# borgor/ripcurrents

Measured on AMD Instinct MI355X. Metric: frames/sec dense Farneback flow @1080p, higher is better.
Workload: dtype f32

## Files before the change

ripcurrents_amd/csrc/flow_iter_kernels.hip:

```cpp

#include <cstdlib>

#include "rc_device.h"

#define RC_ITER_BATCH 3
#define RC_RR_D 3

#ifdef RC_EXACT_BUILD
#define RC_FLOW_NS rc_flow_exact
#else
#define RC_FLOW_NS rc_flow_fast
#endif
namespace RC_FLOW_NS {

__device__ __forceinline__ float2 rc_flow_in(const RcIterArgs& a, const float2* fin, int gx, int gy) {
    if (a.in_mode == 0) return make_float2(0.f, 0.f);
    if (a.in_mode == 1) return fin[(size_t)gy * a.w + gx];
    float ax, ay;
    int sx = rc_src_x(gx, a.up_scale_x, a.fin_w, ax);
    int sx1 = min(sx + 1, a.fin_w - 1);
    int sy = rc_src_y(gy, a.up_scale_y, ay);
    int sy0 = rc_clampi(sy, 0, a.fin_h - 1), sy1 = rc_clampi(sy + 1, 0, a.fin_h - 1);
    const float2* S0 = fin + (size_t)sy0 * a.fin_w;
    const float2* S1 = fin + (size_t)sy1 * a.fin_w;
// ... 10 lines not shown
struct RcM5 { float m0, m1, m2, m3, m4; };

struct RcGather {
    float4 q00, q01, q10, q11;
    float e00, e01, e10, e11;
    float fx, fy;
    bool inside;
};

__device__ __forceinline__ void rc_gather_issue(RcGather& g, const float4* __restrict__ RA1,
                                                const float* __restrict__ RB1, int gx, int gy, float dx,
                                                float dy, int w, int h) {
    float fx = gx + dx, fy = gy + dy;
    int x1 = (int)floorf(fx), y1 = (int)floorf(fy);
    g.fx = fx - x1;
    g.fy = fy - y1;
    g.inside = (unsigned)x1 < (unsigned)(w - 1) && (unsigned)y1 < (unsigned)(h - 1);
    const size_t p = g.inside ? (size_t)y1 * w + x1 : (size_t)gy * w + gx;
    const size_t pw = g.inside ? (size_t)w : 0, p1 = g.inside ? 1 : 0;
    g.q00 = RA1[p]; g.q01 = RA1[p + p1]; g.q10 = RA1[p + pw]; g.q11 = RA1[p + pw + p1];
    g.e00 = RB1[p]; g.e01 = RB1[p + p1]; g.e10 = RB1[p + pw]; g.e11 = RB1[p + pw + p1];
}

__device__ __forceinline__ void rc_r0_prep(float4& A0, float& B0) {
#ifndef RC_EXACT_BUILD
    A0.x *= 0.5f; A0.y *= 0.5f; A0.z *= 0.5f; A0.w *= 0.5f; B0 *= 0.5f;
#endif
}

__device__ __forceinline__ RcM5 rc_matrices_reg(const float4 A0, const float B0, const RcGather& g, float dx,
                                                float dy, int X, int Y, int w, int h, bool BORDER = true) {
    float fx = g.fx, fy = g.fy;
#ifdef RC_EXACT_BUILD
    float a00 = (1.f - fx) * (1.f - fy), a01 = fx * (1.f - fy);
    float a10 = (1.f - fx) * fy, a11 = fx * fy;
#define RC_BILIN(c, e) (a00 * e##00 c + a01 * e##01 c + a10 * e##10 c + a11 * e##11 c)
    float r2 = RC_BILIN(.x, g.q), r3 = RC_BILIN(.y, g.q), r4 = RC_BILIN(.z, g.q), r5 = RC_BILIN(.w, g.q);
    float r6 = RC_BILIN(, g.e);
#undef RC_BILIN
    r4 = (A0.z + r4) * 0.5f;
    r5 = (A0.w + r5) * 0.5f;
    r6 = (B0 + r6) * 0.25f;
    if (!g.inside) {
        r2 = r3 = 0.f;
        r4 = A0.z;
        r5 = A0.w;
        r6 = B0 * 0.5f;
    }
    r2 = (A0.x - r2) * 0.5f;
    r3 = (A0.y - r3) * 0.5f;
#else
    const float hx1 = 0.5f * fx, hx0 = RC_FMA(fx, -0.5f, 0.5f), fy0 = 1.f - fy;
    const float h00 = hx0 * fy0, h01 = hx1 * fy0, h10 = hx0 * fy, h11 = hx1 * fy;
#define RC_BILIN_FROM(s0, sg, c, e) RC_FMA(sg h11, e##11 c, RC_FMA(sg h10, e##10 c, RC_FMA(sg h01, e##01 c, RC_FMA(sg h00, e##00 c, s0))))
    float r2 = RC_BILIN_FROM(A0.x, -, .x, g.q), r3 = RC_BILIN_FROM(A0.y, -, .y, g.q);
    float r4 = RC_BILIN_FROM(A0.z, +, .z, g.q), r5 = RC_BILIN_FROM(A0.w, +, .w, g.q);
    float r6 = 0.5f * RC_BILIN_FROM(B0, +, , g.e);
#undef RC_BILIN_FROM
    if (!g.inside) {
        r2 = A0.x;
        r3 = A0.y;
        r4 = 2.f * A0.z;
        r5 = 2.f * A0.w;
        r6 = B0;
    }
#endif
#ifdef RC_EXACT_BUILD
    r2 += r4 * dy + r6 * dx;
    r3 += r6 * dy + r5 * dx;
#else
    r2 = RC_FMA(r6, dx, RC_FMA(r4, dy, r2));
    r3 = RC_FMA(r5, dx, RC_FMA(r6, dy, r3));
#endif
    if (BORDER && ((unsigned)(X - 5) >= (unsigned)(w - 10) || (unsigned)(Y - 5) >= (unsigned)(h - 10))) {
        float bl = X < 5 ? (X < 2 ? 0.14f : 0.4472f) : 1.f;
        int rx = w - X - 1;
        float br = X >= w - 5 ? (rx < 2 ? 0.14f : 0.4472f) : 1.f;
        float bt = Y < 5 ? (Y < 2 ? 0.14f : 0.4472f) : 1.f;
        int ry = h - Y - 1;
        float bb = Y >= h - 5 ? (ry < 2 ? 0.14f : 0.4472f) : 1.f;
        float scale = bl * br * bt * bb;
        r2 *= scale; r3 *= scale; r4 *= scale; r5 *= scale; r6 *= scale;
    }
    RcM5 o;
#ifdef RC_EXACT_BUILD
    o.m0 = r4 * r4 + r6 * r6;
    o.m1 = (r4 + r5) * r6;
    o.m2 = r5 * r5 + r6 * r6;
    o.m3 = r4 * r2 + r6 * r3;
    o.m4 = r6 * r2 + r5 * r3;
#else
    o.m0 = RC_FMA(r4, r4, r6 * r6);
    o.m1 = (r4 + r5) * r6;
    o.m2 = RC_FMA(r5, r5, r6 * r6);
    o.m3 = RC_FMA(r4, r2, r6 * r3);
    o.m4 = RC_FMA(r6, r2, r5 * r3);
#endif
    return o;
}

__device__ __forceinline__ RcM5 rc_matrices(const float4* __restrict__ RA0, const float* __restrict__ RB0,
                                            const float4* __restrict__ RA1, const float* __restrict__ RB1,
                                            int gx, int gy, int w, int h, float dx, float dy) {
    size_t p0 = (size_t)gy * w + gx;
    float4 A0 = RA0[p0];
    float B0 = RB0[p0];
    RcGather g;
    rc_gather_issue(g, RA1, RB1, gx, gy, dx, dy, w, h);
    rc_r0_prep(A0, B0);
    return rc_matrices_reg(A0, B0, g, dx, dy, gx, gy, w, h);
}

__device__ __forceinline__ float2 rc_solve(const double* g) {
    double idet = 1. / (g[0] * g[2] - g[1] * g[1] + 1e-3);
    float2 f;
    f.x = (float)((g[0] * g[4] - g[1] * g[3]) * idet);
    f.y = (float)((g[2] * g[3] - g[1] * g[4]) * idet);
    return f;
}

__device__ __forceinline__ float rc_diff_of_products(float a, float b, float c, float d) {
    float w = c * d;
    float e = RC_FMA(-c, d, w);
    float f = RC_FMA(a, b, -w);
    return f + e;
}
__device__ __forceinline__ float2 rc_solve3(const float* g, float eps) {
#ifdef RC_EXACT_BUILD
    (void)eps;
    const double d[5] = {g[0], g[1], g[2], g[3], g[4]};
    return rc_solve(d);
#endif
// ... 471 lines not shown
            int sy = rc_src_y(gy[q], a.up_scale_y, ay[q]);
            int sy0 = rc_clampi(sy, 0, a.fin_h - 1), sy1 = rc_clampi(sy + 1, 0, a.fin_h - 1);
            const float2* S0 = fin + (size_t)sy0 * a.fin_w;
            const float2* S1 = fin + (size_t)sy1 * a.fin_w;
            p00[q] = S0[sx]; p01[q] = S0[sx1]; p10[q] = S1[sx]; p11[q] = S1[sx1];
        }
#pragma unroll
        for (int q = 0; q < NIT; q++) {
            float a0 = 1.f - ax[q], a1 = ax[q], b0 = 1.f - ay[q], b1 = ay[q];
            float r0x = p00[q].x * a0 + p01[q].x * a1, r1x = p10[q].x * a0 + p11[q].x * a1;
            float r0y = p00[q].y * a0 + p01[q].y * a1, r1y = p10[q].y * a0 + p11[q].y * a1;
            dx[q] = (r0x * b0 + r1x * b1) * a.up_mul;
            dy[q] = (r0y * b0 + r1y * b1) * a.up_mul;
        }
    }
    float4 A0[NIT];
    float B0[NIT];
    RcGather gt[NIT];
#pragma unroll
    for (int q = 0; q < NIT; q++) {
        size_t p0 = (size_t)gy[q] * w + gx[q];
        A0[q] = RA0[p0];
        B0[q] = RB0[p0];
        rc_r0_prep(A0[q], B0[q]);
        rc_gather_issue(gt[q], RA1, RB1, gx[q], gy[q], dx[q], dy[q], w, h);
    }
#pragma unroll
    for (int q = 0; q < NIT; q++) {
        RcM5 v = rc_matrices_reg(A0[q], B0[q], gt[q], dx[q], dy[q], gx[q], gy[q], w, h);
        int idx = tid + q * RC_W3_THREADS;
        if (idx < NITEMS) {
            int ly = idx / MW, lx = idx - ly * MW;
            float* mp = Ms + ly * MP + lx;
            mp[0] = v.m0;
            mp[MH * MP] = v.m1;
            mp[2 * MH * MP] = v.m2;
            mp[3 * MH * MP] = v.m3;
            mp[4 * MH * MP] = v.m4;
        }
    }
    __syncthreads();

    constexpr int RPT = TH / (RC_W3_THREADS / TW);
    const int lx = tid % TW, r0 = (tid / TW) * RPT;
    const int ox = tx0 + lx;
    float g[RPT][5];
#pragma unroll
// ... 342 lines not shown
    const int ox = tx0 - 2 - D, oy = ty0 - 2 - D;
#define RC_RRC_COORDS(tid_)                                                         \
    const int x = (tid_) & (MW - 1), grp = (tid_) / MW, ly0 = grp * NIT;            \
    const int px = tx0 - 2 + x;                                                     \
    const int gxo = INTERIOR ? px : rc_clampi(px, 0, w - 1);                        \
    int gys[NIT];                                                                   \
    _Pragma("unroll") for (int q = 0; q < NIT; q++)                                 \
        gys[q] = INTERIOR ? ty0 - 2 + ly0 + q : rc_clampi(ty0 - 2 + ly0 + q, 0, h - 1);

    float4 A0[NIT];
    float B0[NIT];
    float dx[NIT], dy[NIT];
    {
        const int tid = threadIdx.x;
        RC_RRC_COORDS(tid)
        const size_t s0 = (size_t)((a.slot0 + zb * a.zstep) % a.nslots) * a.R_slot_stride;
        const size_t s1 = (size_t)((a.slot1 + zb * a.zstep) % a.nslots) * a.R_slot_stride;
        rc_rrc_issue_window<INTERIOR, NT, WP, WN, NWL>(a.RA + s1, a.RB + s1, lds_a, lds_b, tid, ox, oy, w, h);
#pragma unroll
        for (int q = 0; q < NIT; q++) {
            const unsigned p0 = (unsigned)(gys[q] * w + gxo);
            A0[q] = (a.RA + s0)[p0];
            B0[q] = (a.RB + s0)[p0];
            rc_r0_prep(A0[q], B0[q]);
        }
        rc_rr_flow_in<IN_MODE, NIT, MW, MH, INTERIOR>(a, a.fin + (size_t)zb * a.fin_pair_stride, tx0, ty0, gxo, gys, dx, dy);
    }

    for (int z = zb; z < ze; z++) {
        const size_t s1 = (size_t)((a.slot1 + z * a.zstep) % a.nslots) * a.R_slot_stride;
        const float4* __restrict__ RA1 = a.RA + s1;
        const float* __restrict__ RB1 = a.RB + s1;
        const bool more = z + 1 < ze;
        int tid = threadIdx.x;
        asm volatile("" : "+v"(tid));
        RC_RRC_COORDS(tid)
        rc_all_barrier();

        float m[NIT][5];
        rc_rr_matrices<INTERIOR, NIT, WW, WH, WP>(m, A0, B0, dx, dy, LA, LB, ox, oy, RA1, RB1, gxo, gys, w, h);
        rc_rr_exchange<NIT, MW>(m, XR, grp, x);
        rc_lds_barrier();

        {
            float2 f1[NIT];
            rc_rr_flows<GAUSS_, NIT, MW, NG>(m, XR, grp, x, a.win, f1);
            float f1x[NIT], f1y[NIT];
#pragma unroll
            for (int q = 0; q < NIT; q++) { f1x[q] = f1[q].x; f1y[q] = f1[q].y; }
            rc_rr_matrices<INTERIOR, NIT, WW, WH, WP>(m, A0, B0, f1x, f1y, LA, LB, ox, oy, RA1, RB1, gxo, gys, w, h);
        }
        if (more) {
#pragma unroll
            for (int q = 0; q < NIT; q++) {
                const int i = (int)__umul24((unsigned)(gys[q] - oy), (unsigned)WP) + (gxo - ox);
                A0[q] = LA[i];
                B0[q] = LB[i];
                rc_r0_prep(A0[q], B0[q]);
            }
        }
        rc_lds_barrier();
        if constexpr (!INTERIOR) {
#pragma unroll
            for (int q = 0; q < NIT; q++)
#pragma unroll
                for (int c = 0; c < 5; c++) Ms[c * PLANE + (ly0 + q) * MP + x] = m[q][c];
            rc_lds_barrier();
#pragma unroll
            for (int q = 0; q < NIT; q++) {
                const int py = ty0 - 2 + ly0 + q;
                if ((unsigned)px >= (unsigned)w || (unsigned)py >= (unsigned)h) {
                    const int cx = gxo - (tx0 - 2), cy = gys[q] - (ty0 - 2);
#pragma unroll
                    for (int c = 0; c < 5; c++) m[q][c] = Ms[c * PLANE + cy * MP + cx];
                }
            }
        }
        rc_rr_exchange<NIT, MW>(m, XR, grp, x);
        rc_lds_barrier();

        if (more) {
// ... 170 lines not shown
```

ripcurrents_amd/csrc/pyr_polyexp_kernels.hip:

```cpp

#include "rc_device.h"

__global__ __launch_bounds__(RC_BLOCK) void k_pyr_level(RcPyrArgs a) {
    extern __shared__ __align__(16) unsigned char smem[];
    unsigned char* reg = smem;
    float* rp = (float*)(smem + (size_t)a.reg_hmax * a.reg_wp);
    int* xs = (int*)(rp + (size_t)a.reg_hmax * 2 * a.tw);
    float* xa = (float*)(xs + 2 * a.tw);
    int* ys = (int*)(xa + a.tw);
    float* ya = (float*)(ys + 2 * a.th);
    float* ks = ya + a.th;
    const int tid = threadIdx.x, lane = tid & 63, wv = tid >> 6;
    const int z = blockIdx.z;
    const int tx0 = blockIdx.x * a.tw, ty0 = blockIdx.y * a.th;
    const int r = a.ksize >> 1;
    const int W0 = a.W0, H0 = a.H0;

    if (tid < a.tw) {
        float ax;
        int sx = rc_src_x(min(tx0 + tid, a.w - 1), a.scale_x, W0, ax);
        xs[2 * tid] = sx;
        xs[2 * tid + 1] = min(sx + 1, W0 - 1);
        xa[tid] = ax;
    } else if (tid >= 64 && tid < 128) {
// ... 632 lines not shown
    __syncthreads();

    for (int idx = tid; idx < INH * (TW / 4); idx += RC_POLY_BLOCK) {
        int i = idx / (TW / 4), g4 = idx - i * (TW / 4);
        float v[NV];
        {
            const unsigned la = (unsigned)(size_t)((__attribute__((address_space(3))) float*)(tin + i * INW + 4 * g4));
            rc_f32x4 t[NV / 4];
#pragma unroll
            for (int q = 0; q < NV / 4; q++) asm volatile("ds_read_b128 %0, %1 offset:%2" : "=v"(t[q]) : "v"(la), "n"(16 * q));
            if constexpr (NV / 4 == 3) asm volatile("s_waitcnt lgkmcnt(0)" : "+v"(t[0]), "+v"(t[1]), "+v"(t[2]));
            else if constexpr (NV / 4 == 5) asm volatile("s_waitcnt lgkmcnt(0)" : "+v"(t[0]), "+v"(t[1]), "+v"(t[2]), "+v"(t[3]), "+v"(t[4]));
            else {
#pragma unroll
                for (int q = 0; q < NV / 4; q++) asm volatile("s_waitcnt lgkmcnt(0)" : "+v"(t[q]));
            }
#pragma unroll
            for (int q = 0; q < NV / 4; q++) { v[4 * q] = t[q].x; v[4 * q + 1] = t[q].y; v[4 * q + 2] = t[q].z; v[4 * q + 3] = t[q].w; }
        }
        float h0[4], h1[4], h2[4];
#pragma unroll
        for (int p = 0; p < 4; p++) {
            const int c = RP + p;
            float s0 = v[c] * a.pk.g[0], s1 = 0.f, s2 = 0.f;
#pragma unroll
            for (int k = 1; k <= R; k++) {
                float sm = v[c + k] + v[c - k], df = v[c + k] - v[c - k];
                s0 = RC_FMA(sm, a.pk.g[k], s0);
                s1 = RC_FMA(df, a.pk.xg[k], s1);
                s2 = RC_FMA(sm, a.pk.xxg[k], s2);
            }
            h0[p] = s0; h1[p] = s1; h2[p] = s2;
        }
        float4* o = (float4*)(hs + i * TW + 4 * g4);
        o[0] = make_float4(h0[0], h0[1], h0[2], h0[3]);
        o[INH * TW / 4] = make_float4(h1[0], h1[1], h1[2], h1[3]);
        o[2 * INH * TW / 4] = make_float4(h2[0], h2[1], h2[2], h2[3]);
    }
    __syncthreads();

    if constexpr (MFMA) {
        static_assert(TH == 32, "8 waves = 2 x 4 sub-tiles of 16 x 16");
        constexpr int KS = (16 + 2 * R + 3) / 4;
        float* wt = hs + 3 * INH * TW;
        if (tid < 3 * (2 * R + 1)) {
            const int f3 = tid / (2 * R + 1), t = tid - f3 * (2 * R + 1), k = t < R ? R - t : t - R;
            wt[tid] = f3 == 0 ? a.pk.g[k] : (f3 == 1 ? (t < R ? -a.pk.xg[k] : (t == R ? 0.f : a.pk.xg[k])) : a.pk.xxg[k]);
        }
        __syncthreads();
        const int lane = tid & 63, wv = tid >> 6;
        const int i = lane & 15, kk = lane >> 4;
        const int y0 = 16 * (wv >> 2), x0 = 16 * (wv & 3);
        rc_f32x4 c1 = {0, 0, 0, 0}, c2 = c1, c3 = c1, c4 = c1, c5 = c1, c6 = c1;
#pragma unroll
        for (int s = 0; s < KS; s++) {
            const int t = 4 * s + kk - i;
            const bool on = (unsigned)t <= (unsigned)(2 * R);
            const float wg = on ? wt[t] : 0.f, wx = on ? wt[2 * R + 1 + t] : 0.f, wq = on ? wt[2 * (2 * R + 1) + t] : 0.f;
            const int row = min(y0 + 4 * s + kk, INH - 1);
            const float* bp = hs + row * TW + x0 + i;
            const float p0 = bp[0], p1 = bp[INH * TW], p2 = bp[2 * INH * TW];
            c1 = __builtin_amdgcn_mfma_f32_16x16x4f32(wg, p0, c1, 0, 0, 0);
            c3 = __builtin_amdgcn_mfma_f32_16x16x4f32(wx, p0, c3, 0, 0, 0);
            c5 = __builtin_amdgcn_mfma_f32_16x16x4f32(wq, p0, c5, 0, 0, 0);
            c2 = __builtin_amdgcn_mfma_f32_16x16x4f32(wg, p1, c2, 0, 0, 0);
            c6 = __builtin_amdgcn_mfma_f32_16x16x4f32(wx, p1, c6, 0, 0, 0);
            c4 = __builtin_amdgcn_mfma_f32_16x16x4f32(wg, p2, c4, 0, 0, 0);
        }
        const int gx = tx0 + x0 + i;
        if (gx < w) {
            float4* RA = a.RA + (size_t)slot * a.R_slot_stride;
            float* RB = a.RB + (size_t)slot * a.R_slot_stride;
            const double dck = (double)dc * a.pk.kdc;
            const float ig11f = (float)a.pk.ig11, ig55f = (float)a.pk.ig55;
#pragma unroll
            for (int r = 0; r < 4; r++) {
                const int gy = ty0 + y0 + 4 * kk + r;
                if (gy < h) {
                    float4 ra;
                    ra.x = c3[r] * ig11f;
                    ra.y = c2[r] * ig11f;
                    ra.z = (float)((double)c1[r] * a.pk.ig03 + (double)c5[r] * a.pk.ig33 + dck);
                    ra.w = (float)((double)c1[r] * a.pk.ig03 + (double)c4[r] * a.pk.ig33 + dck);
                    size_t p = (size_t)gy * w + gx;
                    RA[p] = ra;
                    RB[p] = c6[r] * ig55f;
                }
            }
        }
        return;
    }
    constexpr int NR = TH / (RC_POLY_BLOCK / 64);
    static_assert(NR * (RC_POLY_BLOCK / 64) == TH, "tile height must be a multiple of 8");
    const int x = tid & 63, o0 = (tid >> 6) * NR;
    constexpr int NW = NR + 2 * R;
    float b1[NR], b2[NR], b3[NR], b4[NR], b5[NR], b6[NR];
    {
        float c[NW];
#pragma unroll
        for (int q = 0; q < NW; q++) c[q] = hs[(o0 + q) * TW + x];
#pragma unroll
        for (int o = 0; o < NR; o++) {
            float s1 = c[o + R] * a.pk.g[0], s3 = 0.f, s5 = 0.f;
#pragma unroll
            for (int k = 1; k <= R; k++) {
                float sm = c[o + R + k] + c[o + R - k], df = c[o + R + k] - c[o + R - k];
                s1 = RC_FMA(sm, a.pk.g[k], s1);
                s3 = RC_FMA(df, a.pk.xg[k], s3);
                s5 = RC_FMA(sm, a.pk.xxg[k], s5);
            }
            b1[o] = s1; b3[o] = s3; b5[o] = s5;
        }
    }
    {
        float c[NW];
#pragma unroll
        for (int q = 0; q < NW; q++) c[q] = hs[INH * TW + (o0 + q) * TW + x];
#pragma unroll
        for (int o = 0; o < NR; o++) {
            float s2 = c[o + R] * a.pk.g[0], s6 = 0.f;
#pragma unroll
            for (int k = 1; k <= R; k++) {
                s2 = RC_FMA(c[o + R + k] + c[o + R - k], a.pk.g[k], s2);
                s6 = RC_FMA(c[o + R + k] - c[o + R - k], a.pk.xg[k], s6);
            }
            b2[o] = s2; b6[o] = s6;
        }
    }
    {
        float c[NW];
#pragma unroll
        for (int q = 0; q < NW; q++) c[q] = hs[2 * INH * TW + (o0 + q) * TW + x];
#pragma unroll
        for (int o = 0; o < NR; o++) {
            float s4 = c[o + R] * a.pk.g[0];
#pragma unroll
            for (int k = 1; k <= R; k++) s4 = RC_FMA(c[o + R + k] + c[o + R - k], a.pk.g[k], s4);
            b4[o] = s4;
        }
    }
    const int gx = tx0 + x;
    if (gx < w) {
        float4* RA = a.RA + (size_t)slot * a.R_slot_stride;
        float* RB = a.RB + (size_t)slot * a.R_slot_stride;
        const double dck = (double)dc * a.pk.kdc;
        const float ig11f = (float)a.pk.ig11, ig55f = (float)a.pk.ig55;
        const float ig03h = (float)a.pk.ig03, ig03l = (float)(a.pk.ig03 - (double)ig03h);
        const float ig33h = (float)a.pk.ig33, ig33l = (float)(a.pk.ig33 - (double)ig33h);
        const float dckh = (float)dck, dckl = (float)(dck - (double)dckh);
#pragma unroll
        for (int o = 0; o < NR; o++) {
            int gy = ty0 + o0 + o;
            if (gy < h) {
                float4 ra;
                ra.x = b3[o] * ig11f;
                ra.y = b2[o] * ig11f;
                const float th = RC_FMA(b1[o], ig03h, dckh), tl = RC_FMA(b1[o], ig03l, dckl);
                ra.z = RC_FMA(b5[o], ig33h, th) + RC_FMA(b5[o], ig33l, tl);
                ra.w = RC_FMA(b4[o], ig33h, th) + RC_FMA(b4[o], ig33l, tl);
                size_t p = (size_t)gy * w + gx;
                __builtin_nontemporal_store(ra.x, &RA[p].x); __builtin_nontemporal_store(ra.y, &RA[p].y);
                __builtin_nontemporal_store(ra.z, &RA[p].z); __builtin_nontemporal_store(ra.w, &RA[p].w);
                __builtin_nontemporal_store(b6[o] * ig55f, &RB[p]);
            }
        }
    }
}

template <int R, int U8, int TH, int MFMA, int PYR = 0>
__global__ __launch_bounds__(RC_POLY_BLOCK) void k_polyexp(RcPolyArgs a) {
    extern __shared__ __align__(16) float rc_poly_smem[];
    rc_polyexp_body<R, U8, TH, MFMA, PYR>(a, blockIdx.x, blockIdx.y, blockIdx.z, rc_poly_smem);
}

template <int R>
__global__ __launch_bounds__(RC_POLY_BLOCK) void k_polyexp_multi(RcPolyArgs a0, RcPolyArgs a1, RcPolyArgs a2, int n0, int n1,
                                                                 int gx0, int gy0, int gx1, int gy1, int gx2, int gy2) {
    extern __shared__ __align__(16) float rc_poly_smem[];
    int id = blockIdx.x;
    if (id < n0) {
        const int z = id / (gx0 * gy0), r = id - z * gx0 * gy0;
        rc_polyexp_body<R, 1, 32, 0>(a0, r % gx0, r / gx0, z, rc_poly_smem);
    } else if (id < n0 + n1) {
        id -= n0;
        const int z = id / (gx1 * gy1), r = id - z * gx1 * gy1;
        rc_polyexp_body<R, 0, 32, 0>(a1, r % gx1, r / gx1, z, rc_poly_smem);
    } else {
        id -= n0 + n1;
        const int z = id / (gx2 * gy2), r = id - z * gx2 * gy2;
        rc_polyexp_body<R, 0, 32, 0>(a2, r % gx2, r / gx2, z, rc_poly_smem);
    }
}

template <int R>
static void launch_polyexp_multi_t(const RcPolyArgs* a, int nlev, int frames, hipStream_t s) {
    constexpr int RP = (R + 3) & ~3;
    constexpr int INW = 64 + 2 * RP, INH = 32 + 2 * R;
    constexpr size_t lds_hs = sizeof(float) * (3 * (size_t)INH * 64 + 3 * (2 * R + 1)), lds_ub = (size_t)(INH + 2) * (INW + 8);
    constexpr size_t lds = sizeof(float) * (size_t)INH * INW + (lds_hs > lds_ub ? lds_hs : lds_ub);
    RC_ALLOW_LDS((k_polyexp_multi<R>), lds);
    int gx[3] = {1, 1, 1}, gy[3] = {1, 1, 1}, n[3] = {0, 0, 0};
    for (int k = 0; k < nlev; k++) { gx[k] = (a[k].w + 63) / 64; gy[k] = (a[k].h + 31) / 32; n[k] = gx[k] * gy[k] * frames; }
    const RcPolyArgs& a2 = nlev > 2 ? a[2] : a[1];
    hipLaunchKernelGGL((k_polyexp_multi<R>), dim3(n[0] + n[1] + n[2]), dim3(RC_POLY_BLOCK), lds, s, a[0], a[1], a2, n[0], n[1],
                       gx[0], gy[0], gx[1], gy[1], gx[2], gy[2]);
}

int rc_polyexp_multi_ok(const RcPolyArgs* a, int nlev) {
    if (nlev < 2 || nlev > 3 || !a[0].src8 || a[0].tile_h != 32 || !a[0].valu_vertical) return 0;
    for (int k = 1; k < nlev; k++) if (a[k].src8 || a[k].pk.n_eff != a[0].pk.n_eff) return 0;
    const int n = a[0].pk.n_eff;
    return n == 3 || n == 5 || n == 7;
}
void rc_launch_polyexp_multi(const RcPolyArgs* a, int nlev, int frames, hipStream_t s) {
    const int n = a[0].pk.n_eff;
    if (n <= 3) launch_polyexp_multi_t<3>(a, nlev, frames, s);
    else if (n <= 5) launch_polyexp_multi_t<5>(a, nlev, frames, s);
    else launch_polyexp_multi_t<7>(a, nlev, frames, s);
}

template <int R, int U8, int TH, int MFMA, int PYR = 0>
static void launch_polyexp_th(const RcPolyArgs& a, int frames, hipStream_t s) {
    constexpr int RP = (R + 3) & ~3;
    constexpr int INW = 64 + 2 * RP, INH = TH + 2 * R;
    constexpr size_t lds_hs = sizeof(float) * (3 * (size_t)INH * 64 + 3 * (2 * R + 1)), lds_ub = (size_t)(INH + 2) * (INW + 8);
    constexpr size_t lds = sizeof(float) * (size_t)INH * INW + (lds_hs > lds_ub ? lds_hs : lds_ub);
    RC_ALLOW_LDS((k_polyexp<R, U8, TH, MFMA, PYR>), lds);
    dim3 grid((a.w + 63) / 64, (a.h + TH - 1) / TH, frames);
    hipLaunchKernelGGL((k_polyexp<R, U8, TH, MFMA, PYR>), grid, dim3(RC_POLY_BLOCK), lds, s, a);
}

template <int R, int U8>
static void launch_polyexp_t(const RcPolyArgs& a, int frames, hipStream_t s) {
    if constexpr (R <= 9) {
        if (a.tile_h == 48) { launch_polyexp_th<R, U8, 48, 0>(a, frames, s); return; }
    }
    if (a.valu_vertical) launch_polyexp_th<R, U8, 32, 0>(a, frames, s);
    else launch_polyexp_th<R, U8, 32, 1>(a, frames, s);
}

template <int U8>
static void launch_polyexp_u(const RcPolyArgs& a, int frames, hipStream_t s) {
    int n = a.pk.n_eff;
    if (n <= 3) launch_polyexp_t<3, U8>(a, frames, s);
    else if (n <= 5) launch_polyexp_t<5, U8>(a, frames, s);
    else if (n <= 7) launch_polyexp_t<7, U8>(a, frames, s);
    else if (n <= 8) launch_polyexp_t<8, U8>(a, frames, s);
    else if (n <= 9) launch_polyexp_t<9, U8>(a, frames, s);
    else if (n <= 12) launch_polyexp_t<12, U8>(a, frames, s);
    else if (n <= 16) launch_polyexp_t<16, U8>(a, frames, s);
    else if (n <= 24) launch_polyexp_t<24, U8>(a, frames, s);
    else launch_polyexp_t<32, U8>(a, frames, s);
}

int rc_polyexp_pyr_ok(const RcPolyArgs& a) {
    const int n = a.pk.n_eff;
    return a.src8 && a.tile_h == 32 && a.valu_vertical && (n == 3 || n == 5 || n == 7);
}

void rc_launch_polyexp(const RcPolyArgs& a, int frames, hipStream_t s) {
    if (a.npyr > 0) {
        const int n = a.pk.n_eff;
        if (n == 3) launch_polyexp_th<3, 1, 32, 0, 1>(a, frames, s);
        else if (n == 5) launch_polyexp_th<5, 1, 32, 0, 1>(a, frames, s);
        else launch_polyexp_th<7, 1, 32, 0, 1>(a, frames, s);
        return;
    }
    if (a.src8) launch_polyexp_u<1>(a, frames, s);
    else launch_polyexp_u<0>(a, frames, s);
}

__global__ void k_pack_R5(const float* R5, float4* RA, float* RB, int n) {
    int i = blockIdx.x * blockDim.x + threadIdx.x;
    if (i < n) {
        RA[i] = make_float4(R5[5 * i], R5[5 * i + 1], R5[5 * i + 2], R5[5 * i + 3]);
        RB[i] = R5[5 * i + 4];
    }
}
__global__ void k_unpack_R5(const float4* RA, const float* RB, float* R5, int n) {
    int i = blockIdx.x * blockDim.x + threadIdx.x;
    if (i < n) {
        float4 v = RA[i];
        R5[5 * i] = v.x; R5[5 * i + 1] = v.y; R5[5 * i + 2] = v.z; R5[5 * i + 3] = v.w;
        R5[5 * i + 4] = RB[i];
    }
}
void rc_launch_pack_R5(const float* R5, float4* RA, float* RB, int n, hipStream_t s) {
    hipLaunchKernelGGL(k_pack_R5, dim3((n + 255) / 256), dim3(256), 0, s, R5, RA, RB, n);
}
void rc_launch_unpack_R5(const float4* RA, const float* RB, float* R5, int n, hipStream_t s) {
    hipLaunchKernelGGL(k_unpack_R5, dim3((n + 255) / 256), dim3(256), 0, s, RA, RB, R5, n);
}
```

ripcurrents_amd/csrc/rc_common.h:

```cpp
#pragma once

#include <hip/hip_runtime.h>
#include <limits.h>
#include <stdint.h>

#include "../../include/rcflow.h"
#include "rc_plan.h"

#define RC_FMA(a, b, c) __builtin_fmaf((a), (b), (c))

__device__ __forceinline__ int rc_cvt_i32_x86(float v) {
    return (v >= -2147483648.f && v < 2147483648.f) ? (int)v : (int)0x80000000;
}

__device__ __forceinline__ const float2* rc_row2(const float* base, size_t step, int y) {
    return (const float2*)((const char*)base + (size_t)y * step);
}

__device__ __forceinline__ bool rc_sample_flow(const float* flow, size_t step, int w, int h, float x, float y,
                                               float& dx, float& dy) {
    int xind = rc_cvt_i32_x86(floorf(x)), yind = rc_cvt_i32_x86(floorf(y));
    float xrem = x - xind, yrem = y - yind;
    if (xind < 1 || yind < 1 || xind + 2 > w || yind + 2 > h) return false;
    const float2* r0 = rc_row2(flow, step, yind) + xind;
// ... 148 lines not shown
    int rc_flow_iter_can_fuse2(const RcIterArgs& a);                          \
    int rc_flow_iter2_r0_reads(const RcIterArgs& a, int pairs);               \
    int rc_flow_chain_groups(const RcIterArgs& a, int pairs, int* starts, int cap); \
    void rc_launch_flow_iter2(const RcIterArgs& a, int pairs, hipStream_t s);
namespace rc_flow_fast { RC_FLOW_DECLS }
namespace rc_flow_exact { RC_FLOW_DECLS }

struct RcFlowAreaArgs {
    const char* src;
    size_t src_step;
    size_t src_pair_stride;
    int W, H;
    float2* dst;
    size_t dst_pair_stride;
    int w, h;
    float mul;
    int fast, ix, iy;
    const int* xstart; const int* xsi; const float* xalpha;
    const int* ystart; const int* ysi; const float* yalpha;
    int lds_tab;
};
void rc_launch_flow_area_init(const RcFlowAreaArgs& a, int pairs, hipStream_t s);

void rc_launch_pack_R5(const float* R5, float4* RA, float* RB, int n, hipStream_t s);
void rc_launch_unpack_R5(const float4* RA, const float* RB, float* R5, int n, hipStream_t s);
```

ripcurrents_amd/csrc/rc_plan.cpp:

```cpp

#include <cfloat>
#include <cmath>
#include <cstring>
#include <vector>

#include "rc_plan.h"

static inline int cv_round(double v) { return (int)nearbyint(v); }

int rc_plan_crop_levels(int w, int h, double pyr_scale, int levels) {
    const int min_size = 32;
    int k;
    double scale = 1;
    for (k = 0; k < levels; k++) {
        scale *= pyr_scale;
        if (w * scale < min_size || h * scale < min_size) break;
    }
    return k;
}

void rc_plan_level_geom(int w, int h, double pyr_scale, int k, RcLevel& L) {
    double scale = 1;
    for (int i = 0; i < k; i++) scale *= pyr_scale;
    L.sigma = (1. / scale - 1) * 0.5;
// ... 98 lines not shown
            t0 += g[k]; t1 += fabs(xg[k]); t2 += xxg[k];
            if (t0 > 1e-8 * (m0 + g[0]) || t1 > 1e-8 * m1 || t2 > 1e-8 * m2) break;
            n_thr = k - 1;
        }
        if (n_thr < 1) n_thr = 1;
    }
    static const int inst[] = {3, 5, 7, 8, 9, 12, 16, 24, 32};
    int R = 32;
    for (int v : inst)
        if (v >= n_thr) { R = v; break; }
    pk.n_eff = R < n ? R : n;
    memset(pk.g, 0, sizeof(pk.g));
    memset(pk.xg, 0, sizeof(pk.xg));
    memset(pk.xxg, 0, sizeof(pk.xxg));
    double sg = 0, s2 = 0;
    for (int k = 0; k <= pk.n_eff; k++) {
        pk.g[k] = g[k];
        pk.xg[k] = xg[k];
        pk.xxg[k] = xxg[k];
        sg += (k ? 2. : 1.) * g[k];
        s2 += (k ? 2. : 0.) * xxg[k];
    }
    pk.kdc = sg * sg * pk.ig03 + sg * s2 * pk.ig33;
    return RC_OK;
}

void rc_plan_window(int winsize, int flags, RcWindow& win) {
    int m = winsize / 2;
    memset(&win, 0, sizeof(win));
    win.m = m;
    win.gaussian = (flags & RC_FARNEBACK_GAUSSIAN) ? 1 : 0;
    win.box_scale = 1. / ((double)winsize * winsize);
    win.box_eps = 1e-3 / (win.box_scale * win.box_scale);
    double sigma = m * 0.3, s = 1;
    win.k[0] = (float)s;
    for (int i = 1; i <= m; i++) {
        float t = (float)exp(-i * i / (2 * sigma * sigma));
        win.k[i] = t;
        s += t * 2;
    }
    s = 1. / s;
    for (int i = 0; i <= m; i++) win.k[i] = (float)(win.k[i] * s);
}

void rc_plan_pick_pyr_tile(RcLevel& L, int W0, int H0) {
    static const int tiles[][2] = {{64, 16}, {64, 8}, {64, 4}, {32, 8}, {16, 8}, {16, 4}, {8, 4}, {4, 4}, {2, 2}, {1, 1}};
// ... 28 lines not shown
```

ripcurrents_amd/csrc/rc_plan.h:

```cpp
#pragma once

#include <stddef.h>

#include "../../include/rcflow.h"

#define RC_MAX_LEVELS 12
#define RC_MAX_POLY_N 32
#define RC_MAX_WIN_M 32

struct RcLevel {
    int w, h;
    double scale_x;
    double scale_y;
    double sigma;
    int ksize;
    int pyr_tw, pyr_th;
    int pyr_reg_w, pyr_reg_h;
    size_t pyr_lds;
};

struct RcPolyK {
    float g[RC_MAX_POLY_N + 1];
    float xg[RC_MAX_POLY_N + 1];
    float xxg[RC_MAX_POLY_N + 1];
    double ig11, ig03, ig33, ig55;
    double kdc;
    int n;
    int n_eff;
};

struct RcWindow {
    float k[RC_MAX_WIN_M + 1];
    double box_scale;
    double box_eps;
    int m;
    int gaussian;
};

int rc_plan_params_valid(const rc_farneback_params* p);
int rc_plan_crop_levels(int w, int h, double pyr_scale, int levels);
void rc_plan_level_geom(int w, int h, double pyr_scale, int k, RcLevel& L);
double rc_plan_scale_pow(double pyr_scale, int L);
void rc_plan_pick_pyr_tile(RcLevel& L, int W0, int H0);
void rc_plan_gaussian_kernel(int n, double sigma, float* cf);
int rc_plan_prepare_poly(int n, double sigma, int exact_taps, RcPolyK& pk);
void rc_plan_window(int winsize, int flags, RcWindow& win);
```

ripcurrents_amd/csrc/rcflow_api.hip:

```cpp

#include <cfloat>
#include <cmath>
#include <cstdarg>
#include <cstdio>
#include <cstring>

#include "rc_host.h"

static thread_local char g_err[512] = "";
void rc_set_error(const char* fmt, ...) {
    va_list ap;
    va_start(ap, fmt);
    vsnprintf(g_err, sizeof(g_err), fmt, ap);
    va_end(ap);
}
extern "C" const char* rcflow_last_error(void) { return g_err; }
extern "C" int rcflow_abi_version(void) { return RCFLOW_ABI_VERSION; }

int rc_buf_ensure(RcBuf& b, size_t bytes) {
    if (b.bytes >= bytes && b.p) return RC_OK;
    if (b.p) (void)hipFree(b.p);
    b.p = nullptr;
    b.bytes = 0;
    if (bytes == 0) return RC_OK;
// ... 272 lines not shown
}

extern "C" int rcflow_debug_level_flow_ptr(rc_ctx* ctx, int stream, int level, int which, float** d_flow, int* w, int* h) {
    RcSlot* s = rc_slot(ctx, stream);
    if (!s || !s->plan.valid || level < 0 || level >= s->plan.nlev || !d_flow) return RC_EINVAL;
    *d_flow = (float*)(which ? s->FB[level].p : s->FA[level].p);
    if (w) *w = s->plan.lv[level].w;
    if (h) *h = s->plan.lv[level].h;
    return *d_flow ? RC_OK : RC_ESTATE;
}

extern "C" int rcflow_debug_plan_poly(int n, double sigma, int exact_taps, float* g, float* xg, float* xxg, double* ig, int* n_eff,
                                      double* kdc) {
    if (n < 1 || n > RC_MAX_POLY_N || !(sigma >= 0) || !g || !xg || !xxg || !ig || !n_eff || !kdc) return RC_EINVAL;
    RcPolyK pk;
    const int rc = rc_plan_prepare_poly(n, sigma, exact_taps, pk);
    if (rc) return rc;
    memcpy(g, pk.g, (n + 1) * sizeof(float));
    memcpy(xg, pk.xg, (n + 1) * sizeof(float));
    memcpy(xxg, pk.xxg, (n + 1) * sizeof(float));
    ig[0] = pk.ig11; ig[1] = pk.ig03; ig[2] = pk.ig33; ig[3] = pk.ig55;
    *n_eff = pk.n_eff;
    *kdc = pk.kdc;
    return RC_OK;
}
extern "C" int rcflow_debug_plan_pyr_kernel(int ksize, double sigma, float* taps) {
    if (ksize < 1 || ksize > 1023 || !(sigma >= 0) || !taps) return RC_EINVAL;
    rc_plan_gaussian_kernel(ksize, sigma, taps);
    return RC_OK;
}
extern "C" int rcflow_debug_kind(int id, const char** name, const char** bucket) {
    if (id < 0 || id >= RC_K_LISTED || !name || !bucket) return RC_EINVAL;
    *name = kKindNames[id];
    *bucket = kBucketNames[kBucketOfKind[id]];
    return RC_OK;
}

extern "C" int rcflow_set_option(rc_ctx* ctx, const char* name, int value) {
    if (!ctx || !name) return RC_EINVAL;
    if (!strcmp(name, "chunk")) {
        if (value < 1 || value > 64) return RC_EINVAL;
        ctx->chunk = value;
    } else if (!strcmp(name, "exact_taps")) {
        ctx->exact_taps = value ? 1 : 0;
    } else if (!strcmp(name, "exact")) {
        if (value < -1 || value > 1) return RC_EINVAL;
// ... 975 lines not shown
    const RcPyrArgs pa = pyr_args(ctx, L, k, d_img, step, 0, w, h, (const float*)s->stage_f32[0].p, d_out, 0, 0, 1, 1);
    rc_launch_pyr(pa, 1, L.pyr_lds, s->cur);
    RC_HIP(hipGetLastError());
    return RC_OK;
}

extern "C" int rcflow_stage_polyexp_dev(rc_ctx* ctx, int stream, const float* d_I, int w, int h, int poly_n,
                                        double poly_sigma, float* d_R5) {
    RcSlot* s = rc_slot(ctx, stream);
    if (!s || !d_I || !d_R5 || w <= 0 || h <= 0 || poly_n < 1 || poly_n > RC_MAX_POLY_N) return RC_EINVAL;
    RC_HIP(hipSetDevice(ctx->device));
    size_t n = (size_t)w * h;
    int rc;
    if ((rc = rc_buf_ensure(s->stage_f32[0], n * sizeof(float4)))) return rc;
    if ((rc = rc_buf_ensure(s->stage_f32[1], n * sizeof(float)))) return rc;
    RcPolyArgs qa;
    memset(&qa, 0, sizeof(qa));
    qa.I = d_I; qa.I_slot_stride = 0;
    qa.RA = (float4*)s->stage_f32[0].p; qa.RB = (float*)s->stage_f32[1].p; qa.R_slot_stride = 0;
    qa.slot0 = 0; qa.nslots = 1; qa.zstep = 1; qa.w = w; qa.h = h; qa.tile_h = ctx->poly_tile_h; qa.valu_vertical = !ctx->poly_mfma;
    if ((rc = rc_plan_prepare_poly(poly_n, poly_sigma, ctx->exact_taps || ctx->exact == 1, qa.pk))) return rc;
    if (ctx->exact == 1) rc_launch_exact_polyexp(qa, 1, s->cur);
    else rc_launch_polyexp(qa, 1, s->cur);
    rc_launch_unpack_R5(qa.RA, qa.RB, d_R5, (int)n, s->cur);
    RC_HIP(hipGetLastError());
    return RC_OK;
}

extern "C" int rcflow_stage_flow_iter_dev(rc_ctx* ctx, int stream, const float* d_R0, const float* d_R1,
                                          const float* d_flow_in, int w, int h, int winsize, int flags,
                                          float* d_flow_out) {
    RcSlot* s = rc_slot(ctx, stream);
    if (!s || !d_R0 || !d_R1 || !d_flow_out || w <= 0 || h <= 0 || winsize < 1 || winsize / 2 > 24 ||
        (flags & ~RC_FARNEBACK_GAUSSIAN))
        return RC_EINVAL;
    RC_HIP(hipSetDevice(ctx->device));
    size_t n = (size_t)w * h;
    int rc;
    if ((rc = rc_buf_ensure(s->stage_f32[0], 2 * n * sizeof(float4)))) return rc;
    if ((rc = rc_buf_ensure(s->stage_f32[1], 2 * n * sizeof(float)))) return rc;
    float4* RA = (float4*)s->stage_f32[0].p;
    float* RB = (float*)s->stage_f32[1].p;
    rc_launch_pack_R5(d_R0, RA, RB, (int)n, s->cur);
    rc_launch_pack_R5(d_R1, RA + n, RB + n, (int)n, s->cur);
    RcWindow win;
    rc_plan_window(winsize, flags, win);
    if (ctx->exact == 1) {
        if ((rc = rc_buf_ensure(s->exM, n * 5 * sizeof(float)))) return rc;
        if ((rc = rc_buf_ensure(s->exV, (size_t)w * ((h + 15) & ~15) * 5 * sizeof(double)))) return rc;
        if ((rc = rc_buf_ensure(s->exG, n * 5 * sizeof(double)))) return rc;
        if ((rc = rc_buf_ensure(s->stage_f32[2], n * sizeof(float2)))) return rc;
        RcExactArgs e;
        memset(&e, 0, sizeof(e));
        e.RA = RA; e.RB = RB; e.n = n; e.slot0 = 0; e.slot1 = 1; e.nslots = 2; e.zstep = 1; e.w = w; e.h = h; e.win = win; e.plain_scans = (ctx->ablate & RC_ABL_EXACT_PLAIN_SCANS) != 0;
        e.flow = (float2*)s->stage_f32[2].p; e.M = (float*)s->exM.p; e.V = s->exV.p; e.G = s->exG.p;
        if (d_flow_in) RC_HIP(hipMemcpyAsync(e.flow, d_flow_in, n * sizeof(float2), hipMemcpyDeviceToDevice, s->cur));
        else RC_HIP(hipMemsetAsync(e.flow, 0, n * sizeof(float2), s->cur));
        rc_launch_exact_matrices(e, 1, s->cur);
        e.out = (char*)d_flow_out; e.out_step = (size_t)w * 8; e.out_pair_stride = n * 8;
        rc_launch_exact_window_solve(e, 1, s->cur);
        RC_HIP(hipGetLastError());
        return RC_OK;
    }
    RcIterArgs a;
    memset(&a, 0, sizeof(a));
    a.RA = RA; a.RB = RB; a.R_slot_stride = n; a.slot0 = 0; a.slot1 = 1; a.nslots = 2; a.zstep = 1;
    a.w = w; a.h = h;
// ... 37 lines not shown
```

Before: 20030.

## Fold polynomial-expansion normalisation constants into filter taps and drop per-pixel scaling

Precomputes scaled filter taps (qh, xga, xgb) on the host so the polyexp kernels no longer multiply by ig11/ig55/ig03/ig33, and the separate g-weighted accumulator (c1/b1) plus its double-precision or hi/lo compensated combine are removed. The stored R coefficients are pre-halved (and RB quartered), so the flow-iteration kernels drop their per-load 0.5 rescale (rc_r0_prep). Pack/unpack helpers gain scale factors to keep the external R5 format unchanged. It trades some float rounding accuracy, since the compensated double-float combine is gone, for fewer MFMA/FMA ops and fewer registers.

New measurement: 20320, median of 6. 1.01x the previous value.

```diff
diff --git a/ripcurrents_amd/csrc/flow_iter_kernels.hip b/ripcurrents_amd/csrc/flow_iter_kernels.hip
--- a/ripcurrents_amd/csrc/flow_iter_kernels.hip
+++ b/ripcurrents_amd/csrc/flow_iter_kernels.hip
@@ -56,11 +56,6 @@
     g.e00 = RB1[p]; g.e01 = RB1[p + p1]; g.e10 = RB1[p + pw]; g.e11 = RB1[p + pw + p1];
 }
 
-__device__ __forceinline__ void rc_r0_prep(float4& A0, float& B0) {
-#ifndef RC_EXACT_BUILD
-    A0.x *= 0.5f; A0.y *= 0.5f; A0.z *= 0.5f; A0.w *= 0.5f; B0 *= 0.5f;
-#endif
-}
 
 __device__ __forceinline__ RcM5 rc_matrices_reg(const float4 A0, const float B0, const RcGather& g, float dx,
                                                 float dy, int X, int Y, int w, int h, bool BORDER = true) {
@@ -84,19 +79,19 @@
     r2 = (A0.x - r2) * 0.5f;
     r3 = (A0.y - r3) * 0.5f;
 #else
-    const float hx1 = 0.5f * fx, hx0 = RC_FMA(fx, -0.5f, 0.5f), fy0 = 1.f - fy;
-    const float h00 = hx0 * fy0, h01 = hx1 * fy0, h10 = hx0 * fy, h11 = hx1 * fy;
+    const float hx0 = 1.f - fx, fy0 = 1.f - fy;
+    const float h00 = hx0 * fy0, h01 = fx * fy0, h10 = hx0 * fy, h11 = fx * fy;
 #define RC_BILIN_FROM(s0, sg, c, e) RC_FMA(sg h11, e##11 c, RC_FMA(sg h10, e##10 c, RC_FMA(sg h01, e##01 c, RC_FMA(sg h00, e##00 c, s0))))
     float r2 = RC_BILIN_FROM(A0.x, -, .x, g.q), r3 = RC_BILIN_FROM(A0.y, -, .y, g.q);
     float r4 = RC_BILIN_FROM(A0.z, +, .z, g.q), r5 = RC_BILIN_FROM(A0.w, +, .w, g.q);
-    float r6 = 0.5f * RC_BILIN_FROM(B0, +, , g.e);
+    float r6 = RC_BILIN_FROM(B0, +, , g.e);
 #undef RC_BILIN_FROM
     if (!g.inside) {
         r2 = A0.x;
         r3 = A0.y;
         r4 = 2.f * A0.z;
         r5 = 2.f * A0.w;
-        r6 = B0;
+        r6 = 2.f * B0;
     }
 #endif
 #ifdef RC_EXACT_BUILD
@@ -141,7 +136,6 @@
     float B0 = RB0[p0];
     RcGather g;
     rc_gather_issue(g, RA1, RB1, gx, gy, dx, dy, w, h);
-    rc_r0_prep(A0, B0);
     return rc_matrices_reg(A0, B0, g, dx, dy, gx, gy, w, h);
 }
 
@@ -659,7 +653,6 @@
         size_t p0 = (size_t)gy[q] * w + gx[q];
         A0[q] = RA0[p0];
         B0[q] = RB0[p0];
-        rc_r0_prep(A0[q], B0[q]);
         rc_gather_issue(gt[q], RA1, RB1, gx[q], gy[q], dx[q], dy[q], w, h);
     }
 #pragma unroll
@@ -1048,7 +1041,6 @@
             const unsigned p0 = (unsigned)(gys[q] * w + gxo);
             A0[q] = (a.RA + s0)[p0];
             B0[q] = (a.RB + s0)[p0];
-            rc_r0_prep(A0[q], B0[q]);
         }
         rc_rr_flow_in<IN_MODE, NIT, MW, MH, INTERIOR>(a, a.fin + (size_t)zb * a.fin_pair_stride, tx0, ty0, gxo, gys, dx, dy);
     }
@@ -1082,7 +1074,6 @@
                 const int i = (int)__umul24((unsigned)(gys[q] - oy), (unsigned)WP) + (gxo - ox);
                 A0[q] = LA[i];
                 B0[q] = LB[i];
-                rc_r0_prep(A0[q], B0[q]);
             }
         }
         rc_lds_barrier();
diff --git a/ripcurrents_amd/csrc/pyr_polyexp_kernels.hip b/ripcurrents_amd/csrc/pyr_polyexp_kernels.hip
--- a/ripcurrents_amd/csrc/pyr_polyexp_kernels.hip
+++ b/ripcurrents_amd/csrc/pyr_polyexp_kernels.hip
@@ -678,13 +678,13 @@
 #pragma unroll
         for (int p = 0; p < 4; p++) {
             const int c = RP + p;
-            float s0 = v[c] * a.pk.g[0], s1 = 0.f, s2 = 0.f;
+            float s0 = v[c] * a.pk.g[0], s1 = 0.f, s2 = v[c] * a.pk.qh[0];
 #pragma unroll
             for (int k = 1; k <= R; k++) {
                 float sm = v[c + k] + v[c - k], df = v[c + k] - v[c - k];
                 s0 = RC_FMA(sm, a.pk.g[k], s0);
-                s1 = RC_FMA(df, a.pk.xg[k], s1);
-                s2 = RC_FMA(sm, a.pk.xxg[k], s2);
+                s1 = RC_FMA(df, a.pk.xga[k], s1);
+                s2 = RC_FMA(sm, a.pk.qh[k], s2);
             }
             h0[p] = s0; h1[p] = s1; h2[p] = s2;
         }
@@ -699,48 +699,48 @@
         static_assert(TH == 32, "8 waves = 2 x 4 sub-tiles of 16 x 16");
         constexpr int KS = (16 + 2 * R + 3) / 4;
         float* wt = hs + 3 * INH * TW;
-        if (tid < 3 * (2 * R + 1)) {
-            const int f3 = tid / (2 * R + 1), t = tid - f3 * (2 * R + 1), k = t < R ? R - t : t - R;
-            wt[tid] = f3 == 0 ? a.pk.g[k] : (f3 == 1 ? (t < R ? -a.pk.xg[k] : (t == R ? 0.f : a.pk.xg[k])) : a.pk.xxg[k]);
+        if (tid < 4 * (2 * R + 1)) {
+            const int f4 = tid / (2 * R + 1), t = tid - f4 * (2 * R + 1), k = t < R ? R - t : t - R;
+            const float odd = f4 == 1 ? a.pk.xga[k] : a.pk.xgb[k];
+            wt[tid] = f4 == 0 ? a.pk.g[k] : (f4 == 2 ? a.pk.qh[k] : (t < R ? -odd : (t == R ? 0.f : odd)));
         }
         __syncthreads();
         const int lane = tid & 63, wv = tid >> 6;
         const int i = lane & 15, kk = lane >> 4;
         const int y0 = 16 * (wv >> 2), x0 = 16 * (wv & 3);
-        rc_f32x4 c1 = {0, 0, 0, 0}, c2 = c1, c3 = c1, c4 = c1, c5 = c1, c6 = c1;
+        rc_f32x4 c2 = {0, 0, 0, 0}, c3 = c2, c4 = c2, c5 = c2, c6 = c2;
 #pragma unroll
         for (int s = 0; s < KS; s++) {
             const int t = 4 * s + kk - i;
             const bool on = (unsigned)t <= (unsigned)(2 * R);
             const float wg = on ? wt[t] : 0.f, wx = on ? wt[2 * R + 1 + t] : 0.f, wq = on ? wt[2 * (2 * R + 1) + t] : 0.f;
+            const float wy = on ? wt[3 * (2 * R + 1) + t] : 0.f;
             const int row = min(y0 + 4 * s + kk, INH - 1);
             const float* bp = hs + row * TW + x0 + i;
             const float p0 = bp[0], p1 = bp[INH * TW], p2 = bp[2 * INH * TW];
-            c1 = __builtin_amdgcn_mfma_f32_16x16x4f32(wg, p0, c1, 0, 0, 0);
             c3 = __builtin_amdgcn_mfma_f32_16x16x4f32(wx, p0, c3, 0, 0, 0);
             c5 = __builtin_amdgcn_mfma_f32_16x16x4f32(wq, p0, c5, 0, 0, 0);
             c2 = __builtin_amdgcn_mfma_f32_16x16x4f32(wg, p1, c2, 0, 0, 0);
-            c6 = __builtin_amdgcn_mfma_f32_16x16x4f32(wx, p1, c6, 0, 0, 0);
+            c6 = __builtin_amdgcn_mfma_f32_16x16x4f32(wy, p1, c6, 0, 0, 0);
             c4 = __builtin_amdgcn_mfma_f32_16x16x4f32(wg, p2, c4, 0, 0, 0);
         }
         const int gx = tx0 + x0 + i;
         if (gx < w) {
             float4* RA = a.RA + (size_t)slot * a.R_slot_stride;
             float* RB = a.RB + (size_t)slot * a.R_slot_stride;
-            const double dck = (double)dc * a.pk.kdc;
-            const float ig11f = (float)a.pk.ig11, ig55f = (float)a.pk.ig55;
+            const float dck = (float)((double)dc * a.pk.kdch);
 #pragma unroll
             for (int r = 0; r < 4; r++) {
                 const int gy = ty0 + y0 + 4 * kk + r;
                 if (gy < h) {
                     float4 ra;
-                    ra.x = c3[r] * ig11f;
-                    ra.y = c2[r] * ig11f;
-                    ra.z = (float)((double)c1[r] * a.pk.ig03 + (double)c5[r] * a.pk.ig33 + dck);
-                    ra.w = (float)((double)c1[r] * a.pk.ig03 + (double)c4[r] * a.pk.ig33 + dck);
+                    ra.x = c3[r];
+                    ra.y = c2[r];
+                    ra.z = c5[r] + dck;
+                    ra.w = c4[r] + dck;
                     size_t p = (size_t)gy * w + gx;
                     RA[p] = ra;
-                    RB[p] = c6[r] * ig55f;
+                    RB[p] = c6[r];
                 }
             }
         }
@@ -750,22 +750,21 @@
     static_assert(NR * (RC_POLY_BLOCK / 64) == TH, "tile height must be a multiple of 8");
     const int x = tid & 63, o0 = (tid >> 6) * NR;
     constexpr int NW = NR + 2 * R;
-    float b1[NR], b2[NR], b3[NR], b4[NR], b5[NR], b6[NR];
+    float b2[NR], b3[NR], b4[NR], b5[NR], b6[NR];
     {
         float c[NW];
 #pragma unroll
         for (int q = 0; q < NW; q++) c[q] = hs[(o0 + q) * TW + x];
 #pragma unroll
         for (int o = 0; o < NR; o++) {
-            float s1 = c[o + R] * a.pk.g[0], s3 = 0.f, s5 = 0.f;
+            float s3 = 0.f, s5 = c[o + R] * a.pk.qh[0];
 #pragma unroll
             for (int k = 1; k <= R; k++) {
                 float sm = c[o + R + k] + c[o + R - k], df = c[o + R + k] - c[o + R - k];
-                s1 = RC_FMA(sm, a.pk.g[k], s1);
-                s3 = RC_FMA(df, a.pk.xg[k], s3);
-                s5 = RC_FMA(sm, a.pk.xxg[k], s5);
-            }
-            b1[o] = s1; b3[o] = s3; b5[o] = s5;
+                s3 = RC_FMA(df, a.pk.xga[k], s3);
+                s5 = RC_FMA(sm, a.pk.qh[k], s5);
+            }
+            b3[o] = s3; b5[o] = s5;
         }
     }
     {
@@ -778,7 +777,7 @@
 #pragma unroll
             for (int k = 1; k <= R; k++) {
                 s2 = RC_FMA(c[o + R + k] + c[o + R - k], a.pk.g[k], s2);
-                s6 = RC_FMA(c[o + R + k] - c[o + R - k], a.pk.xg[k], s6);
+                s6 = RC_FMA(c[o + R + k] - c[o + R - k], a.pk.xgb[k], s6);
             }
             b2[o] = s2; b6[o] = s6;
         }
@@ -799,25 +798,20 @@
     if (gx < w) {
         float4* RA = a.RA + (size_t)slot * a.R_slot_stride;
         float* RB = a.RB + (size_t)slot * a.R_slot_stride;
-        const double dck = (double)dc * a.pk.kdc;
-        const float ig11f = (float)a.pk.ig11, ig55f = (float)a.pk.ig55;
-        const float ig03h = (float)a.pk.ig03, ig03l = (float)(a.pk.ig03 - (double)ig03h);
-        const float ig33h = (float)a.pk.ig33, ig33l = (float)(a.pk.ig33 - (double)ig33h);
-        const float dckh = (float)dck, dckl = (float)(dck - (double)dckh);
+        const float dck = (float)((double)dc * a.pk.kdch);
 #pragma unroll
         for (int o = 0; o < NR; o++) {
             int gy = ty0 + o0 + o;
             if (gy < h) {
                 float4 ra;
-                ra.x = b3[o] * ig11f;
-                ra.y = b2[o] * ig11f;
-                const float th = RC_FMA(b1[o], ig03h, dckh), tl = RC_FMA(b1[o], ig03l, dckl);
-                ra.z = RC_FMA(b5[o], ig33h, th) + RC_FMA(b5[o], ig33l, tl);
-                ra.w = RC_FMA(b4[o], ig33h, th) + RC_FMA(b4[o], ig33l, tl);
+                ra.x = b3[o];
+                ra.y = b2[o];
+                ra.z = b5[o] + dck;
+                ra.w = b4[o] + dck;
                 size_t p = (size_t)gy * w + gx;
                 __builtin_nontemporal_store(ra.x, &RA[p].x); __builtin_nontemporal_store(ra.y, &RA[p].y);
                 __builtin_nontemporal_store(ra.z, &RA[p].z); __builtin_nontemporal_store(ra.w, &RA[p].w);
-                __builtin_nontemporal_store(b6[o] * ig55f, &RB[p]);
+                __builtin_nontemporal_store(b6[o], &RB[p]);
             }
         }
     }
@@ -848,11 +842,12 @@
     }
 }
 
+static_assert(3 * sizeof(RcPolyArgs) + 10 * sizeof(int) <= 4096, "k_polyexp_multi's arguments fit the kernel-argument segment");
 template <int R>
 static void launch_polyexp_multi_t(const RcPolyArgs* a, int nlev, int frames, hipStream_t s) {
     constexpr int RP = (R + 3) & ~3;
     constexpr int INW = 64 + 2 * RP, INH = 32 + 2 * R;
-    constexpr size_t lds_hs = sizeof(float) * (3 * (size_t)INH * 64 + 3 * (2 * R + 1)), lds_ub = (size_t)(INH + 2) * (INW + 8);
+    constexpr size_t lds_hs = sizeof(float) * (3 * (size_t)INH * 64 + 4 * (2 * R + 1)), lds_ub = (size_t)(INH + 2) * (INW + 8);
     constexpr size_t lds = sizeof(float) * (size_t)INH * INW + (lds_hs > lds_ub ? lds_hs : lds_ub);
     RC_ALLOW_LDS((k_polyexp_multi<R>), lds);
     int gx[3] = {1, 1, 1}, gy[3] = {1, 1, 1}, n[3] = {0, 0, 0};
@@ -879,7 +874,7 @@
 static void launch_polyexp_th(const RcPolyArgs& a, int frames, hipStream_t s) {
     constexpr int RP = (R + 3) & ~3;
     constexpr int INW = 64 + 2 * RP, INH = TH + 2 * R;
-    constexpr size_t lds_hs = sizeof(float) * (3 * (size_t)INH * 64 + 3 * (2 * R + 1)), lds_ub = (size_t)(INH + 2) * (INW + 8);
+    constexpr size_t lds_hs = sizeof(float) * (3 * (size_t)INH * 64 + 4 * (2 * R + 1)), lds_ub = (size_t)(INH + 2) * (INW + 8);
     constexpr size_t lds = sizeof(float) * (size_t)INH * INW + (lds_hs > lds_ub ? lds_hs : lds_ub);
     RC_ALLOW_LDS((k_polyexp<R, U8, TH, MFMA, PYR>), lds);
     dim3 grid((a.w + 63) / 64, (a.h + TH - 1) / TH, frames);
@@ -926,24 +921,26 @@
     else launch_polyexp_u<0>(a, frames, s);
 }
 
-__global__ void k_pack_R5(const float* R5, float4* RA, float* RB, int n) {
+__global__ void k_pack_R5(const float* R5, float4* RA, float* RB, int n, float sa, float sb) {
     int i = blockIdx.x * blockDim.x + threadIdx.x;
     if (i < n) {
-        RA[i] = make_float4(R5[5 * i], R5[5 * i + 1], R5[5 * i + 2], R5[5 * i + 3]);
-        RB[i] = R5[5 * i + 4];
-    }
-}
-__global__ void k_unpack_R5(const float4* RA, const float* RB, float* R5, int n) {
+        RA[i] = make_float4(R5[5 * i] * sa, R5[5 * i + 1] * sa, R5[5 * i + 2] * sa, R5[5 * i + 3] * sa);
+        RB[i] = R5[5 * i + 4] * sb;
+    }
+}
+__global__ void k_unpack_R5(const float4* RA, const float* RB, float* R5, int n, float ua, float ub) {
     int i = blockIdx.x * blockDim.x + threadIdx.x;
     if (i < n) {
         float4 v = RA[i];
-        R5[5 * i] = v.x; R5[5 * i + 1] = v.y; R5[5 * i + 2] = v.z; R5[5 * i + 3] = v.w;
-        R5[5 * i + 4] = RB[i];
-    }
-}
-void rc_launch_pack_R5(const float* R5, float4* RA, float* RB, int n, hipStream_t s) {
-    hipLaunchKernelGGL(k_pack_R5, dim3((n + 255) / 256), dim3(256), 0, s, R5, RA, RB, n);
-}
-void rc_launch_unpack_R5(const float4* RA, const float* RB, float* R5, int n, hipStream_t s) {
-    hipLaunchKernelGGL(k_unpack_R5, dim3((n + 255) / 256), dim3(256), 0, s, RA, RB, R5, n);
-}
+        R5[5 * i] = v.x * ua; R5[5 * i + 1] = v.y * ua; R5[5 * i + 2] = v.z * ua; R5[5 * i + 3] = v.w * ua;
+        R5[5 * i + 4] = RB[i] * ub;
+    }
+}
+void rc_launch_pack_R5(const float* R5, float4* RA, float* RB, int n, int fast_scale, hipStream_t s) {
+    hipLaunchKernelGGL(k_pack_R5, dim3((n + 255) / 256), dim3(256), 0, s, R5, RA, RB, n, fast_scale ? 0.5f : 1.f,
+                       fast_scale ? 0.25f : 1.f);
+}
+void rc_launch_unpack_R5(const float4* RA, const float* RB, float* R5, int n, int fast_scale, hipStream_t s) {
+    hipLaunchKernelGGL(k_unpack_R5, dim3((n + 255) / 256), dim3(256), 0, s, RA, RB, R5, n, fast_scale ? 2.f : 1.f,
+                       fast_scale ? 4.f : 1.f);
+}
diff --git a/ripcurrents_amd/csrc/rc_common.h b/ripcurrents_amd/csrc/rc_common.h
--- a/ripcurrents_amd/csrc/rc_common.h
+++ b/ripcurrents_amd/csrc/rc_common.h
@@ -194,5 +194,5 @@
 };
 void rc_launch_flow_area_init(const RcFlowAreaArgs& a, int pairs, hipStream_t s);
 
-void rc_launch_pack_R5(const float* R5, float4* RA, float* RB, int n, hipStream_t s);
-void rc_launch_unpack_R5(const float4* RA, const float* RB, float* R5, int n, hipStream_t s);
+void rc_launch_pack_R5(const float* R5, float4* RA, float* RB, int n, int fast_scale, hipStream_t s);
+void rc_launch_unpack_R5(const float4* RA, const float* RB, float* R5, int n, int fast_scale, hipStream_t s);
diff --git a/ripcurrents_amd/csrc/rc_plan.cpp b/ripcurrents_amd/csrc/rc_plan.cpp
--- a/ripcurrents_amd/csrc/rc_plan.cpp
+++ b/ripcurrents_amd/csrc/rc_plan.cpp
@@ -144,6 +144,16 @@
         s2 += (k ? 2. : 0.) * xxg[k];
     }
     pk.kdc = sg * sg * pk.ig03 + sg * s2 * pk.ig33;
+    memset(pk.qh, 0, sizeof(pk.qh));
+    memset(pk.xga, 0, sizeof(pk.xga));
+    memset(pk.xgb, 0, sizeof(pk.xgb));
+    const double sa = pk.ig11 * 0.5, sb = (pk.ig55 * 0.25) / sa;
+    for (int k = 0; k <= pk.n_eff; k++) {
+        pk.qh[k] = (float)(0.5 * (pk.ig03 * (double)g[k] + pk.ig33 * (double)xxg[k]));
+        pk.xga[k] = (float)((double)xg[k] * sa);
+        pk.xgb[k] = (float)((double)xg[k] * sb);
+    }
+    pk.kdch = 0.5 * pk.kdc;
     return RC_OK;
 }
 
diff --git a/ripcurrents_amd/csrc/rc_plan.h b/ripcurrents_amd/csrc/rc_plan.h
--- a/ripcurrents_amd/csrc/rc_plan.h
+++ b/ripcurrents_amd/csrc/rc_plan.h
@@ -27,6 +27,10 @@
     double kdc;
     int n;
     int n_eff;
+    float qh[RC_MAX_POLY_N + 1];
+    float xga[RC_MAX_POLY_N + 1];
+    float xgb[RC_MAX_POLY_N + 1];
+    double kdch;
 };
 
 struct RcWindow {
diff --git a/ripcurrents_amd/csrc/rcflow_api.hip b/ripcurrents_amd/csrc/rcflow_api.hip
--- a/ripcurrents_amd/csrc/rcflow_api.hip
+++ b/ripcurrents_amd/csrc/rcflow_api.hip
@@ -318,6 +318,17 @@
     ig[0] = pk.ig11; ig[1] = pk.ig03; ig[2] = pk.ig33; ig[3] = pk.ig55;
     *n_eff = pk.n_eff;
     *kdc = pk.kdc;
+    return RC_OK;
+}
+extern "C" int rcflow_debug_plan_poly_folded(int n, double sigma, int exact_taps, float* qh, float* xga, float* xgb, double* kdch) {
+    if (n < 1 || n > RC_MAX_POLY_N || !(sigma >= 0) || !qh || !xga || !xgb || !kdch) return RC_EINVAL;
+    RcPolyK pk;
+    const int rc = rc_plan_prepare_poly(n, sigma, exact_taps, pk);
+    if (rc) return rc;
+    memcpy(qh, pk.qh, (n + 1) * sizeof(float));
+    memcpy(xga, pk.xga, (n + 1) * sizeof(float));
+    memcpy(xgb, pk.xgb, (n + 1) * sizeof(float));
+    *kdch = pk.kdch;
     return RC_OK;
 }
 extern "C" int rcflow_debug_plan_pyr_kernel(int ksize, double sigma, float* taps) {
@@ -1339,7 +1350,7 @@
     if ((rc = rc_plan_prepare_poly(poly_n, poly_sigma, ctx->exact_taps || ctx->exact == 1, qa.pk))) return rc;
     if (ctx->exact == 1) rc_launch_exact_polyexp(qa, 1, s->cur);
     else rc_launch_polyexp(qa, 1, s->cur);
-    rc_launch_unpack_R5(qa.RA, qa.RB, d_R5, (int)n, s->cur);
+    rc_launch_unpack_R5(qa.RA, qa.RB, d_R5, (int)n, ctx->exact != 1, s->cur);
     RC_HIP(hipGetLastError());
     return RC_OK;
 }
@@ -1358,8 +1369,8 @@
     if ((rc = rc_buf_ensure(s->stage_f32[1], 2 * n * sizeof(float)))) return rc;
     float4* RA = (float4*)s->stage_f32[0].p;
     float* RB = (float*)s->stage_f32[1].p;
-    rc_launch_pack_R5(d_R0, RA, RB, (int)n, s->cur);
-    rc_launch_pack_R5(d_R1, RA + n, RB + n, (int)n, s->cur);
+    rc_launch_pack_R5(d_R0, RA, RB, (int)n, ctx->exact != 1, s->cur);
+    rc_launch_pack_R5(d_R1, RA + n, RB + n, (int)n, ctx->exact != 1, s->cur);
     RcWindow win;
     rc_plan_window(winsize, flags, win);
     if (ctx->exact == 1) {
```
